# bobwan1995/cliora

Measured on AMD Instinct MI355X. Metric: sentences/sec (inside+outside fwd+bwd), len-20 d=400 bsz=64, higher is better.
Workload: dtype f32 (compose GEMMs: 3x bf16 MFMA per product, fp32 accumulate)

## Files before the change

### cliora_amd/csrc/api_mlp.hip

```cpp
#include "api_mlp_launch.hpp"
#include "ragged_kernels.hpp"
#include "resident_kernels.hpp"
#include "vl_kernels.hpp"

static bool wavefront_pays(const Plan& p, int env) {
    if (p.L <= 2 || env == 0) return false;
    if (env >= 1) return true;
    const double row_floats_per_level = (double)(p.R_in + p.R_out) / (2.0 * (p.L - 1)) * p.Dp;
    return row_floats_per_level >= 100e3;
}

static bool merged_pays(const Plan& p) {
    if (p.arch != 0 || p.L <= 2) return false;
    if (g_cliora_wavefront != 2 && !(g_cliora_wavefront < 0 && wavefront_pays(p, -1))) return false;
    for (size_t e = 0; e < (size_t)2 * p.L; ++e) {
        const int sp = p.level_geom[e * PLEVEL_INTS + 6];
        if (p.level_geom[e * PLEVEL_INTS + 1] > 0 && !project2_parts_ok(sp)) return false;
    }
    return true;
}

static size_t resident_lds_bytes(const Plan& p) {
    return ((size_t)(p.share ? 7 : 8) * p.Dp * p.Dp + (size_t)RES_WAVES * RES_SCR) * sizeof(float);
}
// ... 488 lines not shown

static int bwd_gemm3_env() {
    static const int shape = gemm3_shape_env("CLIORA_BWD_GEMM3", true);
    return shape;
}
struct BwdCall {
    cliora_plan* plan;
    const cliora_params *P, *G;
    const float *x_span, *obj_span, *drop_mask, *inside_h, *IS, *outside_h, *OS;
    const float *d_inside_h, *d_inside_s, *d_outside_h, *d_outside_s;
    float *ws, *wb, *d_x_span, *d_obj_span;
    int ran_outside;
    hipStream_t st;

    const Plan& p = plan->p;
    const FwdLayout& f = p.fwd;
    const BwdLayout& bw = p.bwd;
    const Dev dv = dev_views(p);
    const int B = p.B, L = p.L, D = p.D, Dp = p.Dp, C = p.C, nb = p.nblk, ldpi = nb * Dp;
    const bool vl = p.R > 0, padded = D != Dp;
    const bool compress = P && P->root_mat;
    const BwdSchedule schedule = compress ? BwdSchedule::OutsideThenInside
                               : resident_pays(plan, vl, compress) ? BwdSchedule::Resident : BwdSchedule::Wavefront;
    const bool resident = schedule == BwdSchedule::Resident;
    const bool two_streams = schedule == BwdSchedule::Wavefront && ran_outside && wavefront_pays(p, g_cliora_wavefront);
    const hipStream_t sb = two_streams ? plan->side : st, sw = plan->side2;
    const float *IH = padded ? ws + f.ihp : inside_h, *OH = padded ? ws + f.ohp : outside_h;
    const float *X = padded ? ws + f.xp : x_span, *OBJ = vl ? (padded ? ws + f.objp : obj_span) : nullptr;
    const float *IHn = vl ? ws + f.att_u : IH, *nrmIn = vl ? ws + f.att_nrmu : ws + f.nrmi;
    float *VH = wb + bw.vh, *dG = wb + bw.dg, *dStot = wb + bw.dstot, *VHo = wb + bw.vh_o, *dGo = wb + bw.dg_o, *dStoto = wb + bw.dstot_o;
    float *DA = wb + bw.da, *DS = wb + bw.ds, *dPI = wb + bw.dpi, *dPO = wb + bw.dpo, *dU = wb + bw.du;
    float *DZ = wb + bw.dz, *Xp = wb + bw.x, *DPP = wb + bw.dpp, *DPB = wb + bw.dpb;
    const float *Sp = ws + f.sp, *Pp = ws + f.pp, *PI = ws + f.pi;
    const uint32_t* YM = reinterpret_cast<const uint32_t*>(ws + f.ymask);
    const bool fuse_dnorm = schedule == BwdSchedule::Wavefront;
    const int gemm3_shape = split_bf16() ? bwd_gemm3_env() : 0;
    const bool tiled = pair_tiles_ok(Dp) && !resident;
    float *sibPL = p.share ? wb + bw.sib_pl : dPI + (size_t)3 * Dp, *sibQL = p.share ? wb + bw.sib_ql : dPI + (size_t)4 * Dp;
    const int ldsib = p.share ? Dp : ldpi;
    const int sib_split = two_streams ? (L * 2) / 5 : 0;

    bool sibling_runs(int s_level) const { return s_level >= 0 && s_level <= p.L - 1 && ran_outside && s_level < sib_split; }

    template <class EP>
    int project_bwd(hipStream_t s, const float* WT, const float* WTfrag, const float* W3s, int K, int ncell, const LevelRowsA& rows, EP ep) const {
        if (gemm3_shape > 0) return launch_rows_direct3x(s, W3s, K, p.Dp, ncell, rows, ep, gemm3_shape);
        return launch_rows_direct(s, WT, WTfrag, IMG_FRAG_F32, K, p.Dp, ncell, rows, ep);
    }
    int project_bwd_level(hipStream_t s, bool outside, const LevelArgs& g, bool fused_norm) const {
        const int ldp = outside ? Dp : ldpi, ncell = B * g.Lc;
        const float *WT = ws + (outside ? f.w1roT : f.wcatT), *WTfrag = ws + (outside ? f.w1roT3 : f.wcatT3), *W3s = ws + (outside ? f.w1roT3s : f.wcatT3s);
        const LevelRowsA rows{outside ? dPO : dPI, ldp, p.C, g.off, g.Lc};
        float* vh = outside ? VHo : VH;
        if (fused_norm)
            return project_bwd(s, WT, WTfrag, W3s, ldp, ncell, rows,
                               NormBwdLevelE{outside ? dGo : dG, vh, outside ? OH : IH, ws + (outside ? f.nrmo : f.nrmi),
                                             wb + (outside ? bw.dots_o : bw.dots), Dp, p.C, g.off, g.Lc, p.normalize});
        return project_bwd(s, WT, WTfrag, W3s, ldp, ncell, rows, StoreLevelE{vh, Dp, p.C, g.off, g.Lc, nullptr, 1});
    }

    int outside_bwd_step(int level, hipEvent_t done) const {
        const LevelArgs g = level_args(p, level, true);
        const int ncell = B * g.Lc;
        const bool fused_norm = fuse_dnorm && level >= 1 && level <= L - 2;
        hipLaunchKernelGGL(cell_gather_bwd_out, dim3(ncell), dim3(256), 0, sb, g, p.D, d_outside_h,
                           level == L - 1 ? nullptr : d_outside_s, dv.use[ROLE_OUTB], DA, DS, PI, ldpi, p.blk_qlo, dPO, VHo, dStoto,
                           OH, ws + f.po, fused_norm ? wb + bw.dots_o : nullptr);
        LAUNCHOK("cell_gather_bwd_out");
        if (level >= 1) OKR(project_bwd_level(sb, true, g, fused_norm));
        if (level == L - 1) {
            if (compress) {
                hipLaunchKernelGGL(cell_dnorm, dim3(cells_grid(ncell)), dim3(256), 0, sb, g, VHo, OH, ws + f.nrmo, p.normalize, dGo);
                LAUNCHOK("cell_dnorm(root)");
                return CLIORA_OK;
            }
            LAUNCH_SIGNALLING(done, root_bwd, dim3(1), dim3(ROOT_WAVES * 64), 0, sb, B, C, Dp, VHo, OH, ws + f.nrmo, p.normalize, wb + bw.groot);
            LAUNCHOK("root_bwd");
            return CLIORA_OK;
        }
        if (!fused_norm) {
            hipLaunchKernelGGL(cell_dnorm, dim3(cells_grid(ncell)), dim3(256), 0, sb, g, VHo, OH, ws + f.nrmo, p.normalize, dGo);
            LAUNCHOK("cell_dnorm(out)");
        }
        {
            ProfScope ps(CLIORA_KCLASS_COMPOSE_BWD, sb);
            OKR(launch_level_compose_bwd(sb, ws + f.w2oT, ws + f.w2oT3, f.S3, Dp, f.ct3, f.ncb3, pair_level(p, level, true), dGo, YM, Pp,
                                         PI + (size_t)p.blk_plo * Dp, ldpi, ws + f.po, Dp, ws + f.b2o, DA, DZ, Xp, DPP, DPB, tiled));
        }
        const int s_level = L - 2 - level;
        const bool sib_last = sibling_runs(s_level);
        LAUNCH_SIGNALLING(sib_last ? nullptr : done, cell_dsoftmax, dim3(cells_grid(ncell)), dim3(256), 0, sb, g, f.ncb3, DPP, DPB, Sp, Pp, OS, dStoto, DS);
        LAUNCHOK("cell_dsoftmax(out)");
        if (sib_last) {
            const LevelArgs gi = level_args(p, s_level, false);
            LAUNCH_SIGNALLING(done, cell_gather_bwd_sib, dim3(B * gi.Lc), dim3(256), 0, sb, gi, dv.use[ROLE_OUTA], DA, DS, OH, sibPL, sibQL, ldsib, wb + bw.sib_s);
            LAUNCHOK("cell_gather_bwd_sib");
        }
        return CLIORA_OK;
    }

    WgradPlacement wgrad_placement() const {
        static const int ksplit_env = [] { const char* e = getenv("CLIORA_WGRAD_SPLIT_LEVEL"); return e ? atoi(e) : -1; }();
        const bool wcat_split_path = split_bf16() && tn_pairs_strided_ok(p.Dp);
        const bool sw_beside = plan->side2_beside;
        WgradPlacement w{};
        w.ksplit = ksplit_env >= 0 ? ksplit_env : !sw_beside ? 0
                 : wcat_split_path ? std::max(1, std::min(2 * L / 5, L - 1)) : std::min(2, L - 1);
        w.tail_cells = p.C;
        static const int early_env = [] { const char* e = getenv("CLIORA_WGRAD_EARLY_STEP"); return e ? atoi(e) : -2; }();
        const int early_auto = L >= 16 && sw_beside ? L / 2 + 1 : -1;
        const int early_pick = early_env == -2 ? early_auto : early_env;
        w.J_early = (p.share && ran_outside && schedule == BwdSchedule::Wavefront && early_pick >= 0 && early_pick <= L - 3) ? early_pick : -1;
        const int early2_pick = L >= 28 ? (w.J_early + L) / 2 : -1;
        w.J_early2 = (w.J_early >= 0 && early2_pick > w.J_early && early2_pick <= L - 3) ? early2_pick : -1;
        return w;
    }
    int wcat_grad(hipStream_t s_, int off, int hi, int accumulate) const {
        if (tn_pairs_strided_ok(Dp) && (long long)B * hi >= 512 && (long long)B * hi < (1LL << 22)) {
            return launch_tn_level_block(s_, dPI, ldpi, IH, B, C, off, hi, Dp, wb + bw.slab2, bw.slab_floats, wb + bw.gwcat, wb + bw.gbcat, accumulate,
                                         std::max(8, (180 / (3 * nb)) / 4 * 4), nb);
        }
        return launch_tn(s_, B * hi, ldpi, Dp, Dp, LevelRowsA{dPI, ldpi, C, off, hi}, LevelRowsA{IH, Dp, C, off, hi}, wb + bw.slab2,
                         bw.slab_floats, wb + bw.gwcat, wb + bw.gbcat, accumulate);
    }
    int pair_rows_early(WgradPlacement& w, int j) const {
// ... 134 lines not shown
                           !ran_outside ? 0 : (level < sib_split ? 1 : 2),
                           sibPL, sibQL, ldsib, wb + bw.sib_s, DA, DS, PI, ldpi, p.share, IH, OH, dPI, VH, dStot,
                           ws + f.bcat, fused_norm ? wb + bw.dots : nullptr);
        LAUNCHOK("cell_gather_bwd_in");
        if (level == 0) {
            HIPOK(hipEventRecord(plan->ev_fork[2], sa));
            w.dpi_done_recorded = true;
        }
        if (level <= L - 2) OKR(project_bwd_level(sa, false, g, fused_norm));
        else if (compress && ran_outside)
            OKR(launch_rows_direct(sa, ws + f.rootwT, PROJ_IMG(f.rootwT3), Dp, Dp, ncell, LevelRowsA{dGo, Dp, C, g.off, g.Lc},
                                   StoreLevelE{VH, Dp, C, g.off, g.Lc, nullptr, 1}));
        if (vl) {
            with_regions(p.R, [&](auto NR) {
                hipLaunchKernelGGL(cell_attend_bwd<decltype(NR)::value>, dim3(ncell), dim3(256), 0, sa, g, VH, IH, ws + f.nrmi, p.normalize, OBJ, p.R,
                                   drop_mask, ws + f.att_pk, wb + bw.dctx, wb + bw.pmo, wb + bw.dsc, IHn, nrmIn, level >= 1 ? dG : (float*)nullptr);
            });
            LAUNCHOK("cell_attend_bwd");
        }
        if (level == w.ksplit && level >= 1) {
            HIPOK(hipEventRecord(plan->ev_fork[2], sa));
            HIPOK(hipStreamWaitEvent(sw, plan->ev_fork[2], 0));
            OKR(wcat_grad(sw, g.off, w.tail_cells - g.off, w.tail_cells < C));
            w.tail_cells = g.off;
        }
        if (level == 0) return CLIORA_OK;
        if (!fused_norm && !vl) {
            hipLaunchKernelGGL(cell_dnorm, dim3(cells_grid(ncell)), dim3(256), 0, sa, g, VH, IHn, nrmIn, p.normalize, dG);
            LAUNCHOK("cell_dnorm(in)");
        }
        {
            ProfScope ps(CLIORA_KCLASS_COMPOSE_BWD, sa);
            OKR(launch_level_compose_bwd(sa, ws + f.w2iT, ws + f.w2iT3, f.S3, Dp, f.ct3, f.ncb3, pair_level(p, level, false), dG, YM, Pp, PI, ldpi,
                                         PI + Dp, ldpi, ws + f.b2i, DA, DZ, Xp, DPP, DPB, tiled));
        }
        hipLaunchKernelGGL(cell_dsoftmax, dim3(cells_grid(ncell)), dim3(256), 0, sa, g, f.ncb3, DPP, DPB, Sp, Pp, IS, dStot, DS);
        LAUNCHOK("cell_dsoftmax(in)");
        if (level == 1 && two_streams) HIPOK(hipEventRecord(plan->ev_join[2], sa));
        return CLIORA_OK;
    }

    int backward_wavefront(WgradPlacement& w) const {
        for (int j = 0; j <= L - 1; ++j) {
            if (ran_outside) OKR(outside_bwd_step(j, two_streams ? plan->ev_level[j] : nullptr));
            if (two_streams && j >= 1) HIPOK(hipStreamWaitEvent(st, plan->ev_level[j - 1], 0));
            OKR(inside_bwd_step(w, L - 1 - j));
            OKR(pair_rows_early(w, j));
        }
        return CLIORA_OK;
    }

    int backward_outside_then_inside(WgradPlacement& w) const {
        for (int j = 0; j <= L - 1 && ran_outside; ++j) OKR(outside_bwd_step(j, nullptr));
        for (int j = 0; j <= L - 1; ++j) OKR(inside_bwd_step(w, L - 1 - j));
        if (ran_outside)
            return launch_tn(st, p.B, Dp, Dp, Dp, LevelRowsA{dGo, Dp, C, C - 1, 1}, LevelRowsA{IH, Dp, C, C - 1, 1}, wb + bw.slab, bw.slab_floats,
                             wb + bw.groot_mat, (float*)nullptr);
        HIPOK(hipMemsetAsync(wb + bw.groot_mat, 0, (size_t)Dp * Dp * sizeof(float), st));
        return CLIORA_OK;
    }

    int backward_resident() const {
        ResArgs a = resident_args(plan, ws, const_cast<float*>(IH), const_cast<float*>(OH), const_cast<float*>(IS), const_cast<float*>(OS), ran_outside);
        a.dIH = d_inside_h; a.dIS = d_inside_s; a.dOH = d_outside_h; a.dOS = d_outside_s;
        a.VHo = VHo; a.dPI = dPI; a.dPO = dPO; a.DA = DA; a.DS = DS; a.DZ = DZ; a.Xrows = Xp; a.dU = dU; a.dX = d_x_span;
        a.trace = res_trace() ? reinterpret_cast<unsigned long long*>(plan->trace_words) : nullptr;
        OKR(cliora_ensure_max_lds((const void*)resident_bwd));
        {
            ProfScope ps(CLIORA_KCLASS_COMPOSE_BWD, st);
            hipLaunchKernelGGL(resident_bwd, dim3(std::min(p.B, std::max(1, plan->ncu))), dim3(RES_THREADS), resident_lds_bytes(p), st, a);
            LAUNCHOK("resident_bwd");
        }
        if (ran_outside) {
            hipLaunchKernelGGL(root_bwd, dim3(1), dim3(ROOT_WAVES * 64), 0, st, p.B, p.C, p.Dp, VHo, OH, ws + f.nrmo, p.normalize, wb + bw.groot);
            LAUNCHOK("root_bwd");
        }
        return CLIORA_OK;
    }
    int run(ForkGuard& fork_guard) const {
        WgradPlacement w = wgrad_placement();
        if (!resident && plan->take_imageless(ws))
            OKR(build_chart_images(plan, ws, compress, st));
        if (two_streams) {
            HIPOK(hipEventRecord(plan->ev_fork[0], st));
            HIPOK(hipStreamWaitEvent(sb, plan->ev_fork[0], 0));
            fork_guard.arm(0, sb, plan->ev_join[0]);
        }
        if (!ran_outside && !p.share)
            HIPOK(hipMemsetAsync(dPI, 0, (size_t)B * C * ldpi * sizeof(float), st));
        if (!ran_outside) {
            HIPOK(hipMemsetAsync(wb + bw.gw2o, 0, (size_t)Dp * Dp * sizeof(float), st));
            HIPOK(hipMemsetAsync(wb + bw.gb2o, 0, (size_t)Dp * sizeof(float), st));
            HIPOK(hipMemsetAsync(wb + bw.gw1ro, 0, (size_t)Dp * Dp * sizeof(float), st));
            HIPOK(hipMemsetAsync(wb + bw.groot, 0, (size_t)Dp * sizeof(float), st));
        }
        switch (schedule) {
            case BwdSchedule::Resident: OKR(backward_resident()); break;
            case BwdSchedule::Wavefront: OKR(backward_wavefront(w)); break;
            case BwdSchedule::OutsideThenInside: OKR(backward_outside_then_inside(w)); break;
        }
        if (!resident) {
            hipLaunchKernelGGL(leaf_bwd_pre, dim3(cells_grid(B * L)), dim3(256), 0, st, B, L, C, Dp, VH, IHn, nrmIn, p.normalize, ws + f.t, dU);
            LAUNCHOK("leaf_bwd_pre");
            if (d_x_span)
                OKR(launch_rows_direct(st, ws + f.wlT, PROJ_IMG(f.wlT3), Dp, Dp, B * L, PlainRowsA{dU, Dp}, StoreRowsE{d_x_span, D, nullptr, 0, D}));
        }
        OKR(weight_grads_tail(w, fork_guard));
        return scatter_grads(w);
    }
};

extern "C" int cliora_chart_backward(cliora_plan* plan, const cliora_params* P, const float* x_span, const float* obj_span,
                                     const float* drop_mask, const float* inside_h, const float* inside_s,
                                     const float* outside_h, const float* outside_s, const float* d_inside_h,
                                     const float* d_inside_s, const float* d_outside_h, const float* d_outside_s,
                                     void* fwd_ws, size_t fwd_ws_bytes, void* bwd_ws, size_t bwd_ws_bytes, float* d_x_span,
                                     float* d_obj_span, const cliora_params* G, int ran_outside, void* stream) {
    if (!plan || !x_span || !inside_h || !inside_s || !outside_h || !outside_s || !fwd_ws || !bwd_ws || !G)
        return fail(CLIORA_EINVAL, "NULL argument");
    const Plan& p = plan->p;
    const bool vl = p.R > 0;
    if (p.arch != 0) return fail(CLIORA_EINVAL, "TreeLSTM plan: use cliora_lstm_backward");
    if (p.is_long()) return fail(CLIORA_EINVAL, "cliora_chart_backward: L > 64 is forward only (cell_dsoftmax, the weight-gradient schedule and the workspace stop at 64 words)");
    if (vl && !obj_span) return fail(CLIORA_EINVAL, "a CLIORA plan (R > 0) needs obj_span");
    if (fwd_ws_bytes < p.fwd.total * sizeof(float)) return fail(CLIORA_ENOMEM, "forward workspace too small");
    if (bwd_ws_bytes < p.bwd.total * sizeof(float)) return fail(CLIORA_ENOMEM, "backward workspace too small");
    if (!plan->uploaded) return fail(CLIORA_EINVAL, "backward called before forward");
    if (vl && d_obj_span && p.Dp > 512) return fail(CLIORA_EINVAL, "obj_grad_reduce: D > 512 is not supported");
    hipStream_t st = (hipStream_t)stream;
    OKR(cliora_plan_ready(plan, st));
    std::lock_guard<std::mutex> lanes_lock(*plan->lanes_mu);
    ForkGuard fork_guard(st);
    fork_guard.arm(1, plan->side2, plan->ev_join[1]);
    return BwdCall{plan, P, G, x_span, obj_span, drop_mask, inside_h, inside_s, outside_h, outside_s, d_inside_h, d_inside_s, d_outside_h, d_outside_s,
                    (float*)fwd_ws, (float*)bwd_ws, d_x_span, d_obj_span, ran_outside, st}.run(fork_guard);
}
```

### cliora_amd/csrc/api_mlp_launch.hpp

```cpp
#pragma once
#include <type_traits>

#include "api_common.hpp"
#include "level_kernels.hpp"

template <int V> using Int = std::integral_constant<int, V>;
template <bool V> using Bool = std::integral_constant<bool, V>;

template <class F>
static auto with_regions(int R, F&& f) {
    return R <= 36 ? f(Int<9>{}) : f(Int<16>{});
}

template <class F>
static int with_compose_shape(int ct, int Dp, F&& f) {
    auto mode = [&](auto CT, auto K16) { return split_bf16() ? f(CT, K16, Bool<false>{}) : f(CT, K16, Bool<true>{}); };
    if (ct == 5 && Dp == 400) return mode(Int<5>{}, Int<25>{});
    switch (ct) {
        case 5: return mode(Int<5>{}, Int<0>{});
        case 4: return mode(Int<4>{}, Int<0>{});
        case 2: return mode(Int<2>{}, Int<0>{});
        default: return mode(Int<1>{}, Int<0>{});
    }
}
// ... 35 lines not shown
        OKR(cliora_ensure_max_lds((const void*)level_compose_fwd<ct_, k16, f32>));
        hipLaunchKernelGGL((level_compose_fwd<ct_, k16, f32>), dim3(sg.gx, ncb), dim3(512), compose_lds_bytes(ct_, S, true), st, sg.Wimg, S, Dp, sg.lv,
                           sg.PA, sg.lda, sg.PB, sg.ldb, sg.bias, Pp, sg.TG, sg.SP, sg.ntask, sg.HP, hp_stride, Dp, ymask, Y);
        LAUNCHOK("level_compose_fwd");
        return CLIORA_OK;
    });
}

static int launch_level_compose2(hipStream_t st, const ComposeSeg& a, const ComposeSeg& b, int S3, int Dp, int ct, int ncb, const float* Pp,
                                 size_t hp_stride, uint32_t* ymask, float* Y) {
    if (a.gx + b.gx <= 0) return CLIORA_OK;
    const int S = compose_image_stride(S3, Dp);
    int gx = a.gx + b.gx;
    if (gx >= 8) gx = (gx + 7) / 8 * 8;
    return with_compose_shape(ct, Dp, [&](auto CT, auto K16, auto F32) {
        constexpr int ct_ = decltype(CT)::value, k16 = decltype(K16)::value;
        constexpr bool f32 = decltype(F32)::value;
        if constexpr (k16 == 25 && !f32) {
            const size_t lds_dual = compose_lds_bytes(ct_, S, true) + (size_t)ct_ * 16 * sizeof(float);
            OKR(cliora_ensure_max_lds((const void*)level_compose_fwd2<ct_, k16, f32, 2>));
            hipLaunchKernelGGL((level_compose_fwd2<ct_, k16, f32, 2>), dim3(gx, ncb), dim3(512), lds_dual, st, a, b, S, Dp, Pp, hp_stride, Dp, ymask, Y);
            LAUNCHOK("level_compose_fwd2(dual)");
        } else {
            OKR(cliora_ensure_max_lds((const void*)level_compose_fwd2<ct_, k16, f32>));
            hipLaunchKernelGGL((level_compose_fwd2<ct_, k16, f32>), dim3(gx, ncb), dim3(512), compose_lds_bytes(ct_, S, true), st, a, b, S, Dp, Pp, hp_stride, Dp, ymask, Y);
            LAUNCHOK("level_compose_fwd2");
        }
        return CLIORA_OK;
    });
}

static int launch_level_compose_bwd(hipStream_t st, const float* WT, const float* WTimg, int S3, int Dp, int ct, int ncb, const PairLevel& lv,
                                    const float* dG, const uint32_t* ymask, const float* Pp, const float* PA, int lda, const float* PB,
                                    int ldb, const float* b2, float* DA, float* DZ, float* X, float* DPP, float* DPB, bool tiled = false, int cus = 256) {
    if (lv.N <= 0 || lv.ncell <= 0) return CLIORA_OK;
    const uint32_t* I = reinterpret_cast<const uint32_t*>(split_bf16() ? WTimg : WT);
    const int S = compose_image_stride(S3, Dp), K = Dp;
    auto launch = [&](auto CT, auto K16, auto F32, auto TILED) {
        constexpr int ct_ = decltype(CT)::value, k16 = decltype(K16)::value;
        constexpr bool f32 = decltype(F32)::value, tiled_ = decltype(TILED)::value;
        OKR(cliora_ensure_max_lds((const void*)level_compose_bwd<ct_, k16, f32, tiled_>));
        const int ntiles = (lv.ncell + 15) / 16 * lv.N;
        const int cap = std::max(1, cus / ncb);
        const int passes = (ntiles + 8 * cap - 1) / (8 * cap);
        int gx = (ntiles + 8 * passes - 1) / (8 * passes);
        if (gx >= 8 && (gx + 7) / 8 * 8 <= cap) gx = (gx + 7) / 8 * 8;
        hipLaunchKernelGGL((level_compose_bwd<ct_, k16, f32, tiled_>), dim3(gx, ncb), dim3(512), compose_lds_bytes(ct_, S, false) + (size_t)((K + 31) / 32 * 32) * sizeof(float), st, I, S, K, lv, dG, ymask,
                           Pp, PA, lda, PB, ldb, b2, K, DA, DZ, X, DPP, DPB);
        LAUNCHOK("level_compose_bwd");
        return CLIORA_OK;
    };
    if (tiled) {
        if (!split_bf16() || ct != 5 || Dp != 400) return fail(CLIORA_EINVAL, "tiled pair-row operands: d = 400 in split-bf16 mode only");
        return launch(Int<5>{}, Int<25>{}, Bool<false>{}, Bool<true>{});
    }
    return with_compose_shape(ct, Dp, [&](auto CT, auto K16, auto F32) { return launch(CT, K16, F32, Bool<false>{}); });
}

static int launch_level_project(hipStream_t st, int SP, const ProjSeg& q, hipEvent_t stop, bool lng) {
    const int nt = q.ntc, nrg = (q.ncell + 15) / 16;
    const int nrgp = nrg >= 8 ? (nrg + 7) / 8 * 8 : nrg;
    auto launch = [&](auto CT, auto SP_, auto LONG) {
        const int ncb = nt / decltype(CT)::value;
        LAUNCH_SIGNALLING(stop, (level_project<decltype(CT)::value, decltype(SP_)::value, decltype(LONG)::value>), dim3(q.sc.nscore + nrgp * ncb),
                          dim3(256), 0, st, q.Wfrag, q.K, nrg, nrgp, ncb, q.ncell, q.Lc, q.C, q.off, q.HP, q.hp_stride, q.normalize, q.bias, q.P,
                          q.ldp, q.H, q.nrm, q.sc);
        LAUNCHOK("level_project");
        return CLIORA_OK;
    };
    const bool wide = nt % 5 == 0 && nrg * (nt / 5) >= KSPLIT_MIN_BLOCKS;
    return with_long(lng, [&](auto LONG) {
        return with_parts(SP, [&](auto SP_) { return wide ? launch(Int<5>{}, SP_, LONG) : launch(Int<1>{}, SP_, LONG); });
    });
}

static int launch_level_project2(hipStream_t st, int SP0, int SP1, const ProjSeg& a, const ProjSeg& b, bool lng) {
    if (!project2_parts_ok(SP0) || !project2_parts_ok(SP1)) return fail(CLIORA_EINVAL, "level_project2: parts per level must be 1, 2 or 4");
    const int n = a.sc.nscore + b.sc.nscore + a.nproj + b.nproj + a.nfin + b.nfin;
    if (n <= 0) return CLIORA_OK;
    return with_long(lng, [&](auto LONG) {
        return with_parts2(SP0, [&](auto S0) {
// ... 9 lines not shown
```

### cliora_amd/csrc/level_kernels.hpp

```cpp
#pragma once
#include <hip/hip_runtime.h>
#include <stdint.h>

#include "chart_kernels.hpp"
#include "wgrad_tiles.hpp"

namespace cliora {

struct PairLevel {
    const int32_t *pa, *pb;
    int Lc, N, C, ncell;
    int rowbase;
    int off;
    long long tilebase;
};

constexpr int LC_SLOTS = 4;

struct StepOperand { u32x4 h, l; };
template <bool F32>
__device__ __forceinline__ StepOperand make_operand(int psrc, const float4& f0, const float4& f1) {
    const float4 a0 = to_mfma_lanes(psrc, f0), a1 = to_mfma_lanes(psrc, f1);
    StepOperand o;
    if constexpr (F32) {
// ... 904 lines not shown
};
constexpr int P2_RT = 1, P2_CT = 1, P2_PD = 4;
template <int SP0, int SP1, bool LONG = false>
__global__ __launch_bounds__(256) void level_project2(ProjSeg a, ProjSeg b) {
    __shared__ float4 part[4][P2_RT * P2_CT][64];
    __shared__ float sh_ss[4][P2_RT * 16];
    int bid = blockIdx.x;
    {
        const int ns = a.sc.nscore + b.sc.nscore, np = a.nproj + b.nproj;
        if (bid < ns + np) bid = bid < np ? bid + ns : bid - np;
    }
    float* sh_sc = LONG ? reinterpret_cast<float*>(&part[0][0][0]) : &sh_ss[0][0];
    if (bid < a.sc.nscore) { score_cell<LONG>(a.sc, cell_of_block(bid, a.sc.g.B, a.sc.g.Lc), sh_sc); return; }
    bid -= a.sc.nscore;
    if (bid < b.sc.nscore) { score_cell<LONG>(b.sc, cell_of_block(bid, b.sc.g.B, b.sc.g.Lc), sh_sc); return; }
    bid -= b.sc.nscore;
    if (bid < a.nproj) {
        project_tile<P2_RT, P2_CT, SP0, P2_PD>(part, sh_ss, bid, a.Wfrag, a.K, a.nrg, a.nrgp, a.ntc,
                                               a.ncell, a.Lc, a.C, a.off, a.HP, a.hp_stride, a.normalize, a.bias, a.P, a.ldp, a.H, a.nrm);
        return;
    }
    bid -= a.nproj;
    if (bid < b.nproj) {
        project_tile<P2_RT, P2_CT, SP1, P2_PD>(part, sh_ss, bid, b.Wfrag, b.K, b.nrg, b.nrgp, b.ntc,
                                               b.ncell, b.Lc, b.C, b.off, b.HP, b.hp_stride, b.normalize, b.bias, b.P, b.ldp, b.H, b.nrm);
        return;
    }
    bid -= b.nproj;
    if (bid < a.nfin) { finish_cells(bid, a.ncell, a.Lc, a.C, a.off, a.K, a.HP, a.hp_stride, a.SPfin, a.normalize, a.H, a.nrm); return; }
    bid -= a.nfin;
    if (bid < b.nfin) finish_cells(bid, b.ncell, b.Lc, b.C, b.off, b.K, b.HP, b.hp_stride, b.SPfin, b.normalize, b.H, b.nrm);
}

template <int CT, int K16, bool F32, bool TILED = false>
__global__ __launch_bounds__(512) void level_compose_bwd(const uint32_t* __restrict__ Wimg, int S_, int K_, PairLevel lv,
                                                         const float* __restrict__ dG, const uint32_t* __restrict__ ymask,
                                                         const float* __restrict__ Pp, const float* __restrict__ PA, int lda,
                                                         const float* __restrict__ PB, int ldb, const float* __restrict__ b2, int Dp,
                                                         float* __restrict__ DA, float* __restrict__ DZ, float* __restrict__ X,
                                                         float* __restrict__ DPP, float* __restrict__ DPB) {
    extern __shared__ __attribute__((aligned(16))) uint32_t lds_img[];
    constexpr int WAVES = 8, T = WAVES * 64, PD = 4;
    constexpr bool KS = K16 > 0;
    constexpr int UNROLL_STEPS = KS ? 64 : 1;
    const int K = KS ? K16 * 16 : K_;
    const int S = F32 ? K : (KS ? (K16 + 1) / 2 * 32 + WS3_PAD : S_);
    const int lane = threadIdx.x & 63;
    const int wave = __builtin_amdgcn_readfirstlane(threadIdx.x >> 6);
    const int i = lane & 15, g = lane >> 4;
    const int li = fetch_row_of(lane), lg = fetch_piece_of(lane), psrc = mfma_src_addr(lane);
    const int fsrc = 4 * (li + 16 * lg);
    const int Kp = F32 ? (K + 31) / 32 * 32 : S - WS3_PAD, half = Kp >> 1;
    const int by = blockIdx.y, gy = gridDim.y;
    const int col0 = by * (CT * 16);
    stage_weight_image(Wimg + (size_t)col0 * S, lds_img, CT * 16 * S, wave, lane, T);
    float* b2s = reinterpret_cast<float*>(lds_img + CT * 16 * S);
    for (int k = threadIdx.x; k < Kp; k += T) b2s[k] = k < K ? b2[k] : 0.f;
    const int nsteps = Kp >> 5;
    const int nsteps_p = (nsteps + PD - 1) / PD * PD;
    int wimg_off = 0;
    const int G = (lv.ncell + 15) >> 4;
    const int ntiles = G * lv.N;
    const int stride = gridDim.x * WAVES;

    struct Ctx { const float* gp; const uint32_t* mp; float* zo; float pn; float* bo; };
    const int NT = Dp >> 4;
    auto rowctx = [&](int tile) {
        const int gt = tile / lv.N, n = tile - gt * lv.N;
        const int t = min(gt * 16 + li, lv.ncell - 1);
        const int b = t / lv.Lc, p = t - b * lv.Lc;
        const size_t prow = (size_t)lv.rowbase + (size_t)t * lv.N + n;
        if (TILED)
            return Ctx{dG + ((size_t)b * lv.C + lv.off + p) * Dp, ymask + prow * gy * 4 + lg,
                       DZ + (size_t)(lv.tilebase + tile) * NT * 256 + 2 * lane, gt * 16 + li < lv.ncell ? Pp[prow] : 0.f, DPB + prow};
        return Ctx{dG + ((size_t)b * lv.C + lv.off + p) * Dp, ymask + prow * gy * 4 + lg, DZ + prow * Dp, Pp[prow], DPB + prow};
    };
    struct Slot { float4 g0, g1; uint32_t m0, m1; };
// ... 54 lines not shown
                    if (second) store_split_tile(zt + 256, make_float4(ctx.pn * f1.x, ctx.pn * f1.y, ctx.pn * f1.z, ctx.pn * f1.w));
                } else {
                    st4(ctx.zo + k, make_float4(ctx.pn * f0.x, ctx.pn * f0.y, ctx.pn * f0.z, ctx.pn * f0.w));
                    if (second) st4(ctx.zo + k + 16, make_float4(ctx.pn * f1.x, ctx.pn * f1.y, ctx.pn * f1.z, ctx.pn * f1.w));
                }
            }
            if (by == 0) {
                bdot += f4dot(f0, *reinterpret_cast<const float4*>(b2s + k));
                if (second) bdot += f4dot(f1, *reinterpret_cast<const float4*>(b2s + k + 16));
            }
            return make_operand<F32>(psrc, f0, f1);
        };
        StepOperand cur = prep(0, ra[0]);
#pragma unroll UNROLL_STEPS
        for (int base = 0; base < nsteps_p; base += PD) {
#pragma unroll
            for (int sl = 0; sl < PD; ++sl) {
                const int st = base + sl;
                if (st < nsteps) {
                    StepOperand nxt = cur;
                    if (st + 1 < nsteps) nxt = prep(st + 1, ra[(sl + 1) % PD]);
                    kstep_mfma<CT, F32>(wimg, i, g, S, half, st, 32 * st + 16 < K, cur, acc);
                    const int nst = st + PD;
                    const bool in_cur = nst < nsteps;
                    issue(sl, pick_pod(in_cur, ctx, ctxn), in_cur ? nst : (sl < nsteps ? sl : 0));
                    __builtin_amdgcn_sched_barrier(0);
                    cur = nxt;
                }
            }
        }
        if (by == 0) {
            bdot += __shfl_xor(bdot, 1);
            bdot += __shfl_xor(bdot, 2);
            if (lg == 0 && gt * 16 + li < lv.ncell) *ctx.bo = bdot;
        }
        float dp = 0.f;
#pragma unroll
        for (int c = 0; c < CT; ++c) {
            const float4 u = to_mfma_lanes(fsrc, make_float4(acc[c][0], acc[c][1], acc[c][2], acc[c][3]));
            const float4 pa4 = ea[c], pb4 = ebv[c];
            const float xs0 = pa4.x + pb4.x, xs1 = pa4.y + pb4.y, xs2 = pa4.z + pb4.z, xs3 = pa4.w + pb4.w;
            const float4 x = make_float4(fmaxf(xs0, 0.f), fmaxf(xs1, 0.f), fmaxf(xs2, 0.f), fmaxf(xs3, 0.f));
            dp = fmaf(u.x, x.x, dp); dp = fmaf(u.y, x.y, dp); dp = fmaf(u.z, x.z, dp); dp = fmaf(u.w, x.w, dp);
            if (ok) {
                const size_t o = prow * Dp + col0 + c * 16 + 4 * lg;
                st4(DA + o, make_float4(x.x > 0.f ? pn * u.x : 0.f, x.y > 0.f ? pn * u.y : 0.f,
                                        x.z > 0.f ? pn * u.z : 0.f, x.w > 0.f ? pn * u.w : 0.f));
                if (!TILED) st4(X + o, x);
            }
            if (TILED)
                store_split_tile(reinterpret_cast<uint32_t*>(X) + ((size_t)(lv.tilebase + tile) * NT + by * CT + c) * 256 + 2 * lane,
                                 ok ? x : f4zero());
        }
        dp += __shfl_xor(dp, 1);
        dp += __shfl_xor(dp, 2);
        if (ok && lg == 0) DPP[prow * gy + by] = dp;
        if (!has_next) break;
        ctx = ctxn;
        tile = ntile;
    }
}

static __global__ __launch_bounds__(256) void cell_dnorm(LevelArgs g, const float* __restrict__ VH, const float* __restrict__ H,
                                                         const float* __restrict__ nrm, int normalize, float* __restrict__ dG) {
    const int lane = threadIdx.x & 63;
    const int t = blockIdx.x * 4 + (threadIdx.x >> 6);
    if (t >= g.B * g.Lc) return;
    const int b = t / g.Lc, p = t - b * g.Lc;
    const size_t crow = (size_t)b * g.C + g.off + p;
    const int Dp = g.Dp, nv = Dp >> 2;
    const bool a0 = lane < nv, a1 = lane + 64 < nv;
    float4 v0 = f4zero(), v1 = f4zero(), h0 = f4zero(), h1 = f4zero();
    if (a0) { v0 = ld4(VH + crow * Dp + 4 * lane); h0 = ld4(H + crow * Dp + 4 * lane); }
    if (a1) { v1 = ld4(VH + crow * Dp + 4 * (lane + 64)); h1 = ld4(H + crow * Dp + 4 * (lane + 64)); }
    unit_norm_bwd(v0, v1, h0, h1, nrm[crow], normalize);
    if (a0) st4(dG + crow * Dp + 4 * lane, v0);
    if (a1) st4(dG + crow * Dp + 4 * (lane + 64), v1);
}

static __global__ __launch_bounds__(256) void cell_dsoftmax(LevelArgs g, int ncb, const float* __restrict__ DPP, const float* __restrict__ DPB,
                                                            const float* __restrict__ Sp, const float* __restrict__ Pp,
                                                            const float* __restrict__ Schart, const float* __restrict__ dStot,
                                                            float* __restrict__ DS) {
    const int lane = threadIdx.x & 63;
    const int t = blockIdx.x * 4 + (threadIdx.x >> 6);
    if (t >= g.B * g.Lc || g.N == 0) return;
    const int b = t / g.Lc, p = t - b * g.Lc;
    const size_t crow = (size_t)b * g.C + g.off + p;
    const size_t row0 = (size_t)g.rowbase + (size_t)t * g.N;
    const bool an = lane < g.N;
    float dp = an ? DPB[row0 + lane] : 0.f;
    if (an)
        for (int cb = 0; cb < ncb; ++cb) dp += DPP[(row0 + lane) * ncb + cb];
    const float pn = an ? Pp[row0 + lane] : 0.f;
    const float sn = an ? Sp[row0 + lane] : 0.f;
    const float mean = wave_sum(pn * dp);
    const float ds = pn * ((dp - mean) + dStot[crow] * (1.f + (sn - Schart[crow])));
    if (an) DS[row0 + lane] = ds;
}

}
```

### cliora_amd/csrc/plan.cpp

```cpp
#include "plan.hpp"

#include <algorithm>

namespace cliora {

static inline int ncells(int L) { return L * (L + 1) / 2; }

static size_t align64(size_t x) { return (x + 63) & ~size_t(63); }

ComposeGeom compose_geom(int ncell, int N, int cap) {
    const int G = (ncell + 15) / 16;
    ComposeGeom best{1, 1, G};
    double best_t = 1e30;
    for (int TG : {1, 2, 4, 8}) {
        const int wpg = 8 / TG;
        const int groups = (G + TG - 1) / TG;
        for (int SP = 1; SP <= HP_PARTS && SP <= std::max(1, N); SP *= 2) {
            const int np = (N + SP - 1) / SP;
            const int ntask = groups * SP;
            const int rounds = (ntask + cap - 1) / cap;
            const int depth = (np + wpg - 1) / wpg;
            const int busy = TG * std::min(wpg, np);
            int simd = depth * (busy > 4 ? 2 : 1);
            if (busy > 4 && wpg == 8 && np % 8 != 0 && np % 8 <= 4) simd -= 1;
// ... 170 lines not shown
            f.ncb3 = nt / f.ct3;
        }
        f.hp = take(arch == 0 ? (size_t)HP_PARTS * BC * Dp : 0);
        f.hp_o = take(arch == 0 ? (size_t)HP_PARTS * BC * Dp : 0);
        f.ymask = take(arch == 0 && !lng ? Rt * f.ncb3 * 4 : 0);
        f.nrmi = take(BC);
        f.nrmo = take(BC);
        f.icp = take(lstm * BC * Dp); f.ocp = take(lstm * BC * Dp);
        f.nrmic = take(lstm * BC); f.nrmoc = take(lstm * BC); f.rootc = take(lstm * Dp);
        f.att_u = take(R > 0 ? BC * Dp : 0);
        f.att_pk = take(R > 0 ? BC * 64 : 0);
        f.att_nrmu = take(R > 0 ? BC : 0);
        f.rootw = take(arch == 0 ? Dp * Dp : 0); f.rootwT = take(arch == 0 ? Dp * Dp : 0);
        f.rootw3 = arch == 0 ? img(Dp, Dp) : o; f.rootwT3 = arch == 0 ? img(Dp, Dp) : o;
        f.rootpb = take(arch == 0 ? (size_t)B * Dp : 0);
        f.total = o;
        f.pair_h = arch == 0 ? o : f.y;
        f.pair_h_floats = arch == 0 && !lng ? align64(Rt * Dp) : 0;
    }
    p.bwd = BwdLayout{};
    if (!lng) {
        BwdLayout& b = p.bwd;
        size_t o = 0;
        auto take = [&](size_t n) { size_t at = o; o = align64(o + n); return at; };
        b.vh = take(BC * Dp); b.dg = take(BC * Dp); b.dstot = take(BC);
        b.vh_o = take(BC * Dp); b.dg_o = take(BC * Dp); b.dstot_o = take(BC);
        b.vc_o = take(lstm * BC * Dp); b.dgc_o = take(lstm * BC * Dp);
        b.da = take(lstm ? 0 : Rt * Dp); b.ds = take(Rt);
        const size_t Rtile = std::max(Rt, (size_t)(p.T_in + p.T_out) * 16);
        b.dz = take(lstm ? 0 : Rtile * Dp);
        b.x = take(arch == 0 ? Rtile * Dp : 0);
        b.dpp = take(arch == 0 ? Rt * p.fwd.ncb3 : 0);
        b.dpb = take(arch == 0 ? Rt : 0);
        b.dcb = take(0); b.vc = take(lstm * BC * Dp); b.dgc = take(lstm * BC * Dp); b.grootc = take(lstm * Dp);
        b.dpi = take(BC * nb * Dp); b.dpo = take(BC * npo * Dp);
        b.dots = take(arch == 0 ? BC : 0); b.dots_o = take(arch == 0 ? BC : 0);
        b.sib_pl = take((arch == 0 && p.share) ? BC * Dp : 0); b.sib_ql = take((arch == 0 && p.share) ? BC * Dp : 0); b.sib_s = take(arch == 0 ? BC : 0);
        b.du = take(BL * nlf * Dp); b.dxp = take(padded ? BL * Dp : 0);
        b.slab_floats = std::max((size_t)2048 * 80 * 80, (size_t)128 * (Dp * Dp + Dp));
        b.slab = take(b.slab_floats);
        b.slab2 = take(arch == 0 ? b.slab_floats : 0);
        b.gwcat = take(nb * Dp * Dp); b.gbcat = take(nb * Dp); b.gw1ro = take(npo * Dp * Dp);
        b.gw2i = take(Dp * Dp); b.gb2i = take(Dp); b.gw2o = take(Dp * Dp); b.gb2o = take(Dp);
        b.gwl = take(nlf * Dp * Dp); b.gbl = take(nlf * Dp); b.groot = take(Dp);
        b.dctx = take(R > 0 ? BC * Dp : 0);
        b.pmo = take(R > 0 ? BC * 64 : 0);
        b.dsc = take(R > 0 ? BC * 64 : 0);
        b.dobjp = take(R > 0 ? (size_t)B * R * Dp : 0);
        b.groot_mat = take(arch == 0 ? Dp * Dp : 0);
        b.total = o;
    }
    {
        auto& v = p.vl;
        size_t o = 0;
        auto take = [&](size_t n) { size_t at = o; o = align64(o + n); return at; };
        v.NRp = ((B * R + 15) / 16) * 16;
        const size_t NR = (size_t)v.NRp;
        const size_t on = R > 0 ? 1 : 0;
        v.oall = take(on * NR * Dp); v.oallT = take(on * NR * Dp);
        v.wall = take(on * NR * Dp); v.wallT = take(on * NR * Dp);
        v.sump = take(on * BC * Dp); v.xwp = take(on * BL * Dp); v.xwn = take(on * BL * Dp); v.dxn = take(on * BL * Dp); v.nrm = take(on * 4 * BL);
        v.gobj = take(on * NR * Dp);
        v.oimg = take(on * NR * ((Dp + 31) / 32 * 32 + 8));
        v.keys = take(on * 2 * (size_t)B * BC);
        v.slab_floats = on * (8 * (NR * Dp) + 64);
        v.slab = take(v.slab_floats);
// ... 98 lines not shown
```

### cliora_amd/csrc/plan.hpp

```cpp
#pragma once
#include <cstddef>
#include <cstdint>
#include <string>
#include <vector>

namespace cliora {

constexpr int ROLE_INA = 0;
constexpr int ROLE_INB = 1;
constexpr int ROLE_OUTA = 2;
constexpr int ROLE_OUTB = 3;
constexpr int N_ROLES = 4;
constexpr int HP_PARTS = 4;
constexpr int CLIORA_MAX_L = 64;
constexpr int CLIORA_MAX_L_FWD = 128;
constexpr int PLEVEL_INTS = 8;

struct UseList {
    std::vector<int32_t> off;
    std::vector<int32_t> row;
    std::vector<int32_t> stride;
    std::vector<int32_t> partner;
};

// ... 5 lines not shown
    size_t w2o, b2o, w2oT;
    size_t w2i3, w2iT3, w2o3, w2oT3;
    int Kp3, S3;
    size_t wl3, wlT3, wcat3, wcatT3, w1ro3, w1roT3;
    size_t wcat3s, wcatT3s, w1ro3s, w1roT3s;
    size_t rootp;
    size_t rootw, rootwT, rootw3, rootwT3, rootpb;
    size_t matp, matq3, qrleaf;
    size_t xp, ihp, ohp;
    size_t objp;
    size_t t;
    size_t pi, po;
    size_t y, x;
    size_t pair_h;
    size_t pair_h_floats;
    size_t sp, pp;
    size_t hp, hp_o;
    size_t ymask;
    int ct3, ncb3;
    size_t nrmi, nrmo;
    size_t icp, ocp, nrmic, nrmoc, rootc;
    size_t att_u, att_pk, att_nrmu;
    size_t total;
};

struct BwdLayout {
    size_t vh, dg, dstot;
    size_t vh_o, dg_o, dstot_o;
    size_t vc_o, dgc_o;
    size_t da, ds;
    size_t dz;
    size_t x;
    size_t dpp, dpb;
    size_t dcb, vc, dgc, grootc;
    size_t dpi, dpo;
    size_t dots, dots_o;
    size_t sib_pl, sib_ql, sib_s;
    size_t du, dxp;
    size_t slab, slab2;
    size_t gwcat, gbcat, gw1ro, gw2i, gb2i, gw2o, gb2o, gwl, gbl, groot, groot_mat;
    size_t dctx, pmo, dsc, dobjp;
    size_t total;
    size_t slab_floats;
};

struct Plan {
    int B, L, D, Dp, C, share, normalize, R;
    int arch;
    int npo, nleaf;
    int off_pr, off_ql;
    int nblk;
    int blk_plo, blk_qlo;
    int P_in, P_out;
    long long R_in, R_out;
    std::vector<int32_t> level_offset;
    std::vector<int32_t> lvl_base_in, lvl_base_out;
    std::vector<int32_t> pair_a_in, pair_b_in;
    std::vector<int32_t> pair_a_out, pair_b_out;
    UseList uses[N_ROLES];
    std::vector<int32_t> arow, brow, trow;
    std::vector<int32_t> level_geom;
    int compose_cap;
    FwdLayout fwd;
    BwdLayout bwd;
    struct VlLayout { size_t oall, oallT, wall, wallT, sump, xwp, xwn, dxn, nrm, gobj, oimg, keys, slab, slab_floats, total; int NRp; } vl;

// ... 29 lines not shown
```

Before: 22110.

## Fuse softmax backward into compose-bwd kernel via last-arriver tile tickets

```diff
diff --git a/cliora_amd/csrc/api_mlp.hip b/cliora_amd/csrc/api_mlp.hip
--- a/cliora_amd/csrc/api_mlp.hip
+++ b/cliora_amd/csrc/api_mlp.hip
@@ -544,6 +544,7 @@
     float *DA = wb + bw.da, *DS = wb + bw.ds, *dPI = wb + bw.dpi, *dPO = wb + bw.dpo, *dU = wb + bw.du;
     float *DZ = wb + bw.dz, *Xp = wb + bw.x, *DPP = wb + bw.dpp, *DPB = wb + bw.dpb;
     const float *Sp = ws + f.sp, *Pp = ws + f.pp, *PI = ws + f.pi;
+    int *arrived_i = reinterpret_cast<int*>(wb + bw.arrived), *arrived_o = arrived_i + bw.arrived_ints;
     const uint32_t* YM = reinterpret_cast<const uint32_t*>(ws + f.ymask);
     const bool fuse_dnorm = schedule == BwdSchedule::Wavefront;
     const int gemm3_shape = split_bf16() ? bwd_gemm3_env() : 0;
@@ -594,15 +595,14 @@
             hipLaunchKernelGGL(cell_dnorm, dim3(cells_grid(ncell)), dim3(256), 0, sb, g, VHo, OH, ws + f.nrmo, p.normalize, dGo);
             LAUNCHOK("cell_dnorm(out)");
         }
+        const int s_level = L - 2 - level;
+        const bool sib_last = sibling_runs(s_level);
         {
             ProfScope ps(CLIORA_KCLASS_COMPOSE_BWD, sb);
             OKR(launch_level_compose_bwd(sb, ws + f.w2oT, ws + f.w2oT3, f.S3, Dp, f.ct3, f.ncb3, pair_level(p, level, true), dGo, YM, Pp,
-                                         PI + (size_t)p.blk_plo * Dp, ldpi, ws + f.po, Dp, ws + f.b2o, DA, DZ, Xp, DPP, DPB, tiled));
-        }
-        const int s_level = L - 2 - level;
-        const bool sib_last = sibling_runs(s_level);
-        LAUNCH_SIGNALLING(sib_last ? nullptr : done, cell_dsoftmax, dim3(cells_grid(ncell)), dim3(256), 0, sb, g, f.ncb3, DPP, DPB, Sp, Pp, OS, dStoto, DS);
-        LAUNCHOK("cell_dsoftmax(out)");
+                                         PI + (size_t)p.blk_plo * Dp, ldpi, ws + f.po, Dp, ws + f.b2o, DA, DZ, Xp, DPP, DPB, Sp, OS, dStoto, DS,
+                                         arrived_o, sib_last ? nullptr : done, tiled));
+        }
         if (sib_last) {
             const LevelArgs gi = level_args(p, s_level, false);
             LAUNCH_SIGNALLING(done, cell_gather_bwd_sib, dim3(B * gi.Lc), dim3(256), 0, sb, gi, dv.use[ROLE_OUTA], DA, DS, OH, sibPL, sibQL, ldsib, wb + bw.sib_s);
@@ -803,10 +803,8 @@
         {
             ProfScope ps(CLIORA_KCLASS_COMPOSE_BWD, sa);
             OKR(launch_level_compose_bwd(sa, ws + f.w2iT, ws + f.w2iT3, f.S3, Dp, f.ct3, f.ncb3, pair_level(p, level, false), dG, YM, Pp, PI, ldpi,
-                                         PI + Dp, ldpi, ws + f.b2i, DA, DZ, Xp, DPP, DPB, tiled));
-        }
-        hipLaunchKernelGGL(cell_dsoftmax, dim3(cells_grid(ncell)), dim3(256), 0, sa, g, f.ncb3, DPP, DPB, Sp, Pp, IS, dStot, DS);
-        LAUNCHOK("cell_dsoftmax(in)");
+                                         PI + Dp, ldpi, ws + f.b2i, DA, DZ, Xp, DPP, DPB, Sp, IS, dStot, DS, arrived_i, nullptr, tiled));
+        }
         if (level == 1 && two_streams) HIPOK(hipEventRecord(plan->ev_join[2], sa));
         return CLIORA_OK;
     }
@@ -852,6 +850,7 @@
         WgradPlacement w = wgrad_placement();
         if (!resident && plan->take_imageless(ws))
             OKR(build_chart_images(plan, ws, compress, st));
+        if (!resident) HIPOK(hipMemsetAsync(arrived_i, 0, (size_t)2 * bw.arrived_ints * sizeof(int), st));
         if (two_streams) {
             HIPOK(hipEventRecord(plan->ev_fork[0], st));
             HIPOK(hipStreamWaitEvent(sb, plan->ev_fork[0], 0));
@@ -892,7 +891,7 @@
     const Plan& p = plan->p;
     const bool vl = p.R > 0;
     if (p.arch != 0) return fail(CLIORA_EINVAL, "TreeLSTM plan: use cliora_lstm_backward");
-    if (p.is_long()) return fail(CLIORA_EINVAL, "cliora_chart_backward: L > 64 is forward only (cell_dsoftmax, the weight-gradient schedule and the workspace stop at 64 words)");
+    if (p.is_long()) return fail(CLIORA_EINVAL, "cliora_chart_backward: L > 64 is forward only (the softmax backward, the weight-gradient schedule and the workspace stop at 64 words)");
     if (vl && !obj_span) return fail(CLIORA_EINVAL, "a CLIORA plan (R > 0) needs obj_span");
     if (fwd_ws_bytes < p.fwd.total * sizeof(float)) return fail(CLIORA_ENOMEM, "forward workspace too small");
     if (bwd_ws_bytes < p.bwd.total * sizeof(float)) return fail(CLIORA_ENOMEM, "backward workspace too small");
diff --git a/cliora_amd/csrc/api_mlp_launch.hpp b/cliora_amd/csrc/api_mlp_launch.hpp
--- a/cliora_amd/csrc/api_mlp_launch.hpp
+++ b/cliora_amd/csrc/api_mlp_launch.hpp
@@ -91,8 +91,13 @@
 
 static int launch_level_compose_bwd(hipStream_t st, const float* WT, const float* WTimg, int S3, int Dp, int ct, int ncb, const PairLevel& lv,
                                     const float* dG, const uint32_t* ymask, const float* Pp, const float* PA, int lda, const float* PB,
-                                    int ldb, const float* b2, float* DA, float* DZ, float* X, float* DPP, float* DPB, bool tiled = false, int cus = 256) {
-    if (lv.N <= 0 || lv.ncell <= 0) return CLIORA_OK;
+                                    int ldb, const float* b2, float* DA, float* DZ, float* X, float* DPP, float* DPB, const float* Sp,
+                                    const float* Schart, const float* dStot, float* DS, int* arrived, hipEvent_t done, bool tiled = false,
+                                    int cus = 256) {
+    if (lv.N <= 0 || lv.ncell <= 0) {
+        if (done) HIPOK(hipEventRecord(done, st));
+        return CLIORA_OK;
+    }
     const uint32_t* I = reinterpret_cast<const uint32_t*>(split_bf16() ? WTimg : WT);
     const int S = compose_image_stride(S3, Dp), K = Dp;
     auto launch = [&](auto CT, auto K16, auto F32, auto TILED) {
@@ -104,8 +109,9 @@
         const int passes = (ntiles + 8 * cap - 1) / (8 * cap);
         int gx = (ntiles + 8 * passes - 1) / (8 * passes);
         if (gx >= 8 && (gx + 7) / 8 * 8 <= cap) gx = (gx + 7) / 8 * 8;
-        hipLaunchKernelGGL((level_compose_bwd<ct_, k16, f32, tiled_>), dim3(gx, ncb), dim3(512), compose_lds_bytes(ct_, S, false) + (size_t)((K + 31) / 32 * 32) * sizeof(float), st, I, S, K, lv, dG, ymask,
-                           Pp, PA, lda, PB, ldb, b2, K, DA, DZ, X, DPP, DPB);
+        LAUNCH_SIGNALLING(done, (level_compose_bwd<ct_, k16, f32, tiled_>), dim3(gx, ncb), dim3(512),
+                          compose_lds_bytes(ct_, S, false) + (size_t)((K + 31) / 32 * 32) * sizeof(float), st, I, S, K, lv, dG, ymask,
+                          Pp, PA, lda, PB, ldb, b2, K, DA, DZ, X, DPP, DPB, Sp, Schart, dStot, DS, arrived);
         LAUNCHOK("level_compose_bwd");
         return CLIORA_OK;
     };
diff --git a/cliora_amd/csrc/level_kernels.hpp b/cliora_amd/csrc/level_kernels.hpp
--- a/cliora_amd/csrc/level_kernels.hpp
+++ b/cliora_amd/csrc/level_kernels.hpp
@@ -960,17 +960,60 @@
     if (bid < b.nfin) finish_cells(bid, b.ncell, b.Lc, b.C, b.off, b.K, b.HP, b.hp_stride, b.SPfin, b.normalize, b.H, b.nrm);
 }
 
+__device__ __forceinline__ float ld_agent(const float* p) { return __hip_atomic_load(p, __ATOMIC_RELAXED, __HIP_MEMORY_SCOPE_AGENT); }
+__device__ __forceinline__ void st_agent(float* p, float v) { __hip_atomic_store(p, v, __ATOMIC_RELAXED, __HIP_MEMORY_SCOPE_AGENT); }
+template <int NCB>
+struct SoftmaxBwdCell { float dp, part[NCB > 0 ? NCB : 1], pn, sn, dstot, stot; };
+template <int NCB>
+__device__ __forceinline__ SoftmaxBwdCell<NCB> softmax_bwd_load(const PairLevel& lv, int t, int lane, int ncb, const float* DPP, const float* DPB,
+                                                                const float* __restrict__ Sp, const float* __restrict__ Pp,
+                                                                const float* __restrict__ Schart, const float* __restrict__ dStot) {
+    const int b = t / lv.Lc, p = t - b * lv.Lc;
+    const size_t crow = (size_t)b * lv.C + lv.off + p;
+    const size_t row = (size_t)lv.rowbase + (size_t)t * lv.N + min(lane, lv.N - 1);
+    SoftmaxBwdCell<NCB> c;
+    c.dp = ld_agent(DPB + row);
+    if constexpr (NCB > 0) {
+#pragma unroll
+        for (int cb = 0; cb < NCB; ++cb) c.part[cb] = ld_agent(DPP + row * NCB + cb);
+    } else {
+        for (int cb = 0; cb < ncb; ++cb) c.dp += ld_agent(DPP + row * ncb + cb);
+    }
+    c.pn = Pp[row];
+    c.sn = Sp[row];
+    c.dstot = dStot[crow];
+    c.stot = Schart[crow];
+    return c;
+}
+template <int NCB>
+__device__ __forceinline__ void softmax_bwd_finish(const PairLevel& lv, int t, int lane, const SoftmaxBwdCell<NCB>& c, float* __restrict__ DS) {
+    const bool an = lane < lv.N;
+    float dp = c.dp;
+    if constexpr (NCB > 0) {
+#pragma unroll
+        for (int cb = 0; cb < NCB; ++cb) dp += c.part[cb];
+    }
+    if (!an) dp = 0.f;
+    const float pn = an ? c.pn : 0.f, sn = an ? c.sn : 0.f;
+    const float mean = wave_sum(pn * dp);
+    const float ds = pn * ((dp - mean) + c.dstot * (1.f + (sn - c.stot)));
+    if (an) DS[(size_t)lv.rowbase + (size_t)t * lv.N + lane] = ds;
+}
+
 template <int CT, int K16, bool F32, bool TILED = false>
 __global__ __launch_bounds__(512) void level_compose_bwd(const uint32_t* __restrict__ Wimg, int S_, int K_, PairLevel lv,
                                                          const float* __restrict__ dG, const uint32_t* __restrict__ ymask,
                                                          const float* __restrict__ Pp, const float* __restrict__ PA, int lda,
                                                          const float* __restrict__ PB, int ldb, const float* __restrict__ b2, int Dp,
                                                          float* __restrict__ DA, float* __restrict__ DZ, float* __restrict__ X,
-                                                         float* __restrict__ DPP, float* __restrict__ DPB) {
+                                                         float* DPP, float* DPB, const float* __restrict__ Sp,
+                                                         const float* __restrict__ Schart, const float* __restrict__ dStot,
+                                                         float* __restrict__ DS, int* arrived) {
     extern __shared__ __attribute__((aligned(16))) uint32_t lds_img[];
     constexpr int WAVES = 8, T = WAVES * 64, PD = 4;
     constexpr bool KS = K16 > 0;
     constexpr int UNROLL_STEPS = KS ? 64 : 1;
+    constexpr int DSM_CELLS = 8;
     const int K = KS ? K16 * 16 : K_;
     const int S = F32 ? K : (KS ? (K16 + 1) / 2 * 32 + WS3_PAD : S_);
     const int lane = threadIdx.x & 63;
@@ -1091,7 +1134,7 @@
         if (by == 0) {
             bdot += __shfl_xor(bdot, 1);
             bdot += __shfl_xor(bdot, 2);
-            if (lg == 0 && gt * 16 + li < lv.ncell) *ctx.bo = bdot;
+            if (lg == 0 && gt * 16 + li < lv.ncell) st_agent(ctx.bo, bdot);
         }
         float dp = 0.f;
 #pragma unroll
@@ -1113,7 +1156,26 @@
         }
         dp += __shfl_xor(dp, 1);
         dp += __shfl_xor(dp, 2);
-        if (ok && lg == 0) DPP[prow * gy + by] = dp;
+        if (ok && lg == 0) st_agent(DPP + prow * gy + by, dp);
+        asm volatile("s_waitcnt vmcnt(0)" ::: "memory");
+        int ticket = 0;
+        if (lane == 0) ticket = __hip_atomic_fetch_add(arrived + gt, 1, __ATOMIC_RELAXED, __HIP_MEMORY_SCOPE_AGENT);
+        ticket = __builtin_amdgcn_readfirstlane(ticket);
+        if (ticket == lv.N * gy - 1) {
+            __builtin_amdgcn_fence(__ATOMIC_ACQUIRE, "agent");
+            constexpr int NCB = KS ? K16 / CT : 0;
+            for (int c0 = 0; c0 < 16 && gt * 16 + c0 < lv.ncell; c0 += DSM_CELLS) {
+                SoftmaxBwdCell<NCB> cell[DSM_CELLS];
+#pragma unroll
+                for (int c = 0; c < DSM_CELLS; ++c)
+                    cell[c] = softmax_bwd_load<NCB>(lv, min(gt * 16 + c0 + c, lv.ncell - 1), lane, gy, DPP, DPB, Sp, Pp, Schart, dStot);
+                __builtin_amdgcn_sched_barrier(0);
+#pragma unroll
+                for (int c = 0; c < DSM_CELLS; ++c)
+                    if (gt * 16 + c0 + c < lv.ncell) softmax_bwd_finish(lv, gt * 16 + c0 + c, lane, cell[c], DS);
+            }
+            if (lane == 0) __hip_atomic_store(arrived + gt, 0, __ATOMIC_RELAXED, __HIP_MEMORY_SCOPE_AGENT);
+        }
         if (!has_next) break;
         ctx = ctxn;
         tile = ntile;
@@ -1137,25 +1199,4 @@
     if (a1) st4(dG + crow * Dp + 4 * (lane + 64), v1);
 }
 
-static __global__ __launch_bounds__(256) void cell_dsoftmax(LevelArgs g, int ncb, const float* __restrict__ DPP, const float* __restrict__ DPB,
-                                                            const float* __restrict__ Sp, const float* __restrict__ Pp,
-                                                            const float* __restrict__ Schart, const float* __restrict__ dStot,
-                                                            float* __restrict__ DS) {
-    const int lane = threadIdx.x & 63;
-    const int t = blockIdx.x * 4 + (threadIdx.x >> 6);
-    if (t >= g.B * g.Lc || g.N == 0) return;
-    const int b = t / g.Lc, p = t - b * g.Lc;
-    const size_t crow = (size_t)b * g.C + g.off + p;
-    const size_t row0 = (size_t)g.rowbase + (size_t)t * g.N;
-    const bool an = lane < g.N;
-    float dp = an ? DPB[row0 + lane] : 0.f;
-    if (an)
-        for (int cb = 0; cb < ncb; ++cb) dp += DPP[(row0 + lane) * ncb + cb];
-    const float pn = an ? Pp[row0 + lane] : 0.f;
-    const float sn = an ? Sp[row0 + lane] : 0.f;
-    const float mean = wave_sum(pn * dp);
-    const float ds = pn * ((dp - mean) + dStot[crow] * (1.f + (sn - Schart[crow])));
-    if (an) DS[row0 + lane] = ds;
-}
-
-}
+}
diff --git a/cliora_amd/csrc/plan.cpp b/cliora_amd/csrc/plan.cpp
--- a/cliora_amd/csrc/plan.cpp
+++ b/cliora_amd/csrc/plan.cpp
@@ -226,6 +226,8 @@
         b.x = take(arch == 0 ? Rtile * Dp : 0);
         b.dpp = take(arch == 0 ? Rt * p.fwd.ncb3 : 0);
         b.dpb = take(arch == 0 ? Rt : 0);
+        b.arrived_ints = arch == 0 ? (BL + 15) / 16 : 0;
+        b.arrived = take(2 * b.arrived_ints);
         b.dcb = take(0); b.vc = take(lstm * BC * Dp); b.dgc = take(lstm * BC * Dp); b.grootc = take(lstm * Dp);
         b.dpi = take(BC * nb * Dp); b.dpo = take(BC * npo * Dp);
         b.dots = take(arch == 0 ? BC : 0); b.dots_o = take(arch == 0 ? BC : 0);
diff --git a/cliora_amd/csrc/plan.hpp b/cliora_amd/csrc/plan.hpp
--- a/cliora_amd/csrc/plan.hpp
+++ b/cliora_amd/csrc/plan.hpp
@@ -61,6 +61,7 @@
     size_t dz;
     size_t x;
     size_t dpp, dpb;
+    size_t arrived, arrived_ints;
     size_t dcb, vc, dgc, grootc;
     size_t dpi, dpo;
     size_t dots, dots_o;
```

New measurement: 20730. -6.3%, worse.
